# AlexanderVeselov/RayTracing

Measured on AMD Instinct MI355X. Metric: Mrays/s (all bounces+shadow), higher is better.
Workload: dtype f32

## Files before the change

### raytracing_amd/csrc/frame_kernels.h

```cpp
#pragma once
#include "raygen_kernels.h"
#include "trace_kernels.h"
#include "shade_kernels.h"

#define RT_FRAME_COUNT_STRIDE 136u

struct FrameArgs
{
    ShadeArgs shade;
    float4* o4[2]; float4* d4[2]; float4* thr[2];
    float4* hits;
    float4* sh_o4; float4* sh_d4; uint32_t* sh_aux;
    float4* radiance;
    uint2* spill;
    uint32_t* slow_list;
    uint32_t* wave_counts;
    rt_camera cam;
    float tan_half_fov;
    uint32_t max_bounces, drop_last, tune, tail_q, chunks_per_wave;
};

#ifndef RT_FRAME_WAVES
#define RT_FRAME_WAVES 5
#endif
// ... 51 lines not shown
        if (lane == 0) row[bounce] = n;
        if (lane == 0) row[130] = 0;
        w4_trace_body<false, 12, false, true, true>(sc, fa.o4[cur], fa.d4[cur], (const uint32_t*)nullptr, n, (uint32_t*)nullptr, fa.hits, log, fa.spill,
            fa.tune, my_slow, row + 130, row + 128, (unsigned long long*)nullptr, 0u, 0u, fa.tail_q, 1u, stack, w, G, first, S);
        {
            __threadfence_block();
            const uint32_t n_slow = row[130];
            for (uint32_t k = lane; k < n_slow; k += 64u)
            {
                const uint32_t i = my_slow[k];
                float4 hit;
                (void)v1_trace_ray<false>(sc, fa.o4[cur][i], fa.d4[cur][i], spill_push, spill_pop, hit);
                fa.hits[i] = hit;
            }
            if (lane == 0 && n_slow != 0u) row[129] += n_slow;
            __threadfence_block();
        }
        const unsigned long long t1 = wall_clock64();
        t_closest += t1 - t0;
        ShadeArgs a = fa.shade;
        a.in_o4 = fa.o4[cur]; a.in_d4 = fa.d4[cur]; a.in_thr = fa.thr[cur]; a.hits = fa.hits;
        a.bounce = bounce;
        a.emit_outgoing = (fa.drop_last && bounce >= fa.max_bounces) ? 0u : 1u;
        a.final_bounce = bounce >= fa.max_bounces ? 1u : 0u;
        a.count_in_ray = 1u;
        uint32_t n_next = 0, n_shadow = 0;
        for (uint32_t base = 0; base < n; base += 64u)
        {
            const uint32_t p = base + lane;
            bool want_shadow = false, want_next = false, no_block = false;
            uint32_t next_flag = 0, sh_entry = 0;
            float4 sh_o = make_float4(0, 0, 0, 0), sh_d = sh_o, nx_o = sh_o, nx_d = sh_o, nx_t = sh_o;
            if (p < n)
                shade_entry<FURNACE, BLUE, false, false>(sc, tile, a, index_of(p), want_shadow, want_next, no_block, next_flag, sh_o, sh_d, nx_o, nx_d, nx_t, sh_entry);
            const unsigned long long ms = __ballot(want_shadow), mn = __ballot(want_next);
            const unsigned long long lt = (1ull << lane) - 1ull;
            if (want_shadow)
            {
                const uint32_t i = index_of(n_shadow + (uint32_t)__popcll(ms & lt));
                fa.sh_o4[i] = sh_o; fa.sh_d4[i] = sh_d; fa.sh_aux[i] = sh_entry;
            }
            if (want_next)
            {
                const uint32_t i = index_of(n_next + (uint32_t)__popcll(mn & lt));
                fa.o4[cur ^ 1u][i] = nx_o; fa.d4[cur ^ 1u][i] = nx_d; fa.thr[cur ^ 1u][i] = nx_t;
            }
            n_shadow += (uint32_t)__popcll(ms);
            n_next += (uint32_t)__popcll(mn);
        }
        __threadfence_block();
        const unsigned long long t2 = wall_clock64();
        t_shade += t2 - t1;
        if (lane == 0) row[64u + bounce] = n_shadow;
        if (n_shadow != 0u)
        {
            if (lane == 0) row[130] = 0;
            w4_trace_body<true, 12, false, true, true>(sc, fa.sh_o4, fa.sh_d4, fa.sh_aux, n_shadow, (uint32_t*)nullptr, (float4*)nullptr, log, fa.spill,
                fa.tune, my_slow, row + 130, row + 128, (unsigned long long*)nullptr, 0u, 0u, fa.tail_q, 1u, stack, w, G, first, S);
            __threadfence_block();
            const uint32_t n_slow = row[130];
            for (uint32_t k = lane; k < n_slow; k += 64u)
            {
                const uint32_t i = my_slow[k];
                const float4 rd = fa.sh_d4[i];
                float4 hit;
                if (v1_trace_ray<true>(sc, fa.sh_o4[i], rd, spill_push, spill_pop, hit)) log_retract(log, fa.sh_aux[i], __float_as_uint(rd.w));
            }
            if (lane == 0 && n_slow != 0u) row[129] += n_slow;
            __threadfence_block();
        }
        t_shadow += wall_clock64() - t2;
        cur ^= 1u;
        n = n_next;
        if (n == 0u) break;
    }
    if (lane == 0)
    {
        row[131] = (uint32_t)t_closest; row[132] = (uint32_t)t_shade; row[133] = (uint32_t)t_shadow; row[134] = (uint32_t)(wall_clock64() - t_begin);
    }
    for (uint32_t p = lane; p < n_pixels; p += 64u)
    {
        const uint32_t id = index_of(p);
        const uint32_t c = log.cnt[id];
        if (c == 0u) continue;
        float4 r = fa.radiance[id];
        for (uint32_t k = 0; k < c; ++k)
        {
            const rt_rgb v = *reinterpret_cast<const rt_rgb*>(log.rlog + 3 * ((size_t)k * log.stride + id));
            r.x += v.x; r.y += v.y; r.z += v.z;
        }
        log.cnt[id] = 0;
        fa.radiance[id] = r;
    }
}

__global__ __launch_bounds__(256) void k_frame_sum(const uint32_t* __restrict__ wave_counts, uint32_t n_waves, uint32_t bounces, DCounters* __restrict__ counters)
{
    __shared__ uint32_t part[256];
    const uint32_t col = blockIdx.x;
    uint32_t s = 0;
    for (uint32_t wv = threadIdx.x; wv < n_waves; wv += 256u) s += wave_counts[(size_t)wv * RT_FRAME_COUNT_STRIDE + col];
    part[threadIdx.x] = s;
    __syncthreads();
    for (uint32_t step = 128u; step != 0u; step >>= 1)
    {
        if (threadIdx.x < step) part[threadIdx.x] += part[threadIdx.x + step];
        __syncthreads();
    }
    if (threadIdx.x == 0)
    {
        if (col < 64u) { if (col <= bounces) counters->queue[col] = part[0]; }
        else if (col < 128u) { if (col - 64u <= bounces) counters->shadow[col - 64u] = part[0]; }
        else if (col == 128u) counters->stack_spills += part[0];
        else counters->slow_rays += part[0];
    }
}
```

### raytracing_amd/csrc/kernels_common.h

```cpp
#pragma once
#include "device_math.h"
#include "rt_types.h"

#define RT_LEAF_BIT 0x80000000u
#define RT_EMPTY_REF 0xFFFFFFFFu
#define RT_TRACE_STACK_LDS 24
#define RT_TRACE_STACK_MAX 64

struct rt_rgb { float x, y, z; };
RT_DEV void log_store(float* __restrict__ rlog, size_t index, float x, float y, float z)
{
    rt_rgb v = {x, y, z};
    *reinterpret_cast<rt_rgb*>(rlog + 3 * index) = v;
}

typedef float rt_v4f __attribute__((ext_vector_type(4)));
RT_DEV float4 q_load(const float4* p) { const rt_v4f t = __builtin_nontemporal_load((const rt_v4f*)p); return make_float4(t.x, t.y, t.z, t.w); }
RT_DEV void q_store(float4* p, const float4& v) { const rt_v4f t = {v.x, v.y, v.z, v.w}; __builtin_nontemporal_store(t, (rt_v4f*)p); }

struct DLog
{
    float* rlog;
    uint32_t* cnt;
    uint32_t* ovf_slot;
    uint32_t stride;
    uint32_t inline_entries;
    uint32_t ovf_blocks;
};
RT_DEV size_t log_index(const DLog& L, uint32_t k, uint32_t id, uint32_t slot)
{
    if (k < L.inline_entries) return (size_t)k * L.stride + id;
    if (slot >= L.ovf_blocks) return ~(size_t)0;
    return (size_t)L.inline_entries * L.stride + (size_t)(k - L.inline_entries) * L.ovf_blocks + slot;
}
RT_DEV void log_put(const DLog& L, uint32_t k, uint32_t id, uint32_t slot, float x, float y, float z)
{
    const size_t i = log_index(L, k, id, slot);
    if (i != ~(size_t)0) log_store(L.rlog, i, x, y, z);
}

struct DScene
{
    const float4* nodes;
    const float4* tris_rt;
    const float4* tris_sh;
    const rt_packed_material* materials;
    const rt_texture* textures;
    const uint32_t* texture_data;
    const float4* lights;
    const float4* env;
    const float* gamma_lut;
    int env_w, env_h;
    uint32_t light_count;
    uint32_t root_ref;
    uint32_t entry_ref;
    const float4* wnodes;
    uint32_t w_entry_ref;
    const float4* wnodes_sh;
    uint32_t w_sh_entry_ref;
    float root_min[3];
    float root_max[3];
    const uint16_t* mat_tex16;
    const uint32_t* emissive;
    uint32_t emissive_count;
    uint32_t emissive_nee;
};

struct DTile
{
    uint32_t width, height;
// ... 39 lines not shown
```

### raytracing_amd/csrc/rt_hip.hip

```cpp
#include <hip/hip_runtime.h>
#include <stdio.h>
#include <stdlib.h>
#include <string.h>
#include <math.h>
#include <cmath>
#include <algorithm>
#include <string>
#include <vector>
#include <map>
#include <thread>
#include <atomic>
#include <array>
#include "rt_hip.h"
#include "kernels.h"
#include "own_bvh.h"
#include "treelet_order.h"
#include "tree_select.h"
#include "tree_rotate.h"
#include <chrono>
#include "wide_bvh.h"
#include "device_fold.h"
#include "refit.h"
#include "filters_host.h"
using namespace rtw;
// ... 1101 lines not shown
    HIPCHK(f->ctx, hipStreamWaitEvent(f->p->stream, f->p->ev_shadow[q], 0));
    f->p->shadow_in_flight[q] = false;
    return RT_OK;
}

bool side_on(const rt_frame* f) { return f->overlap_shadow != 0 && !(f->denoiser || f->aov != 0); }

int ensure_slots(rt_frame* f, uint32_t want)
{
    uint32_t cap = slot_cap(f);
    if (want > cap) want = cap;
    if (want <= f->slots && 2u * (f->max_bounces + 1u) <= f->log_entries && f->chunk_pixels == chunk_for(f, f->slots) &&
        (f->log_ovf_blocks != 0u) == log_is_compact(f, f->slots))
        return RT_OK;
    if (flush_log(f) != RT_OK || join_pipes(f) != RT_OK) return RT_ERROR;
    HIPCHK(f->ctx, hipStreamSynchronize(f->ctx->stream));
    uint32_t keep = f->slots < cap ? f->slots : cap;
    uint32_t n = want > keep ? want : keep;
    while (alloc_path_buffers(f, n) != RT_OK)
    {
        if (n == 1) return RT_ERROR;
        n = n > 2u * keep && keep > 0 ? n / 2u : (n > keep ? keep : n / 2u);
        if (n == 0) n = 1;
        f->slots_limit = n;
    }
    return RT_OK;
}

DLog dlog(const rt_frame* f)
{
    DLog L;
    L.rlog = f->p->rlog; L.cnt = f->p->cnt; L.ovf_slot = f->log_ovf_blocks ? f->p->ovf_slot : nullptr;
    L.stride = f->log_stride; L.inline_entries = f->log_inline; L.ovf_blocks = f->log_ovf_blocks;
    return L;
}

int ensure_whole_tile(rt_frame* f)
{
    if (f->chunk_pixels >= (f->n_local ? f->n_local : 1u)) return RT_OK;
    if (f->p->cur_slots != 0) return fail(f->ctx, "rt_generate_rays: the previous sample was not advanced (rt_advance_sample)");
    if (flush_log(f) != RT_OK || join_pipes(f) != RT_OK) return RT_ERROR;
    HIPCHK(f->ctx, hipStreamSynchronize(f->ctx->stream));
    return alloc_path_buffers(f, 1);
}

int flush_log(rt_frame* f, bool keep_open)
{
    rt_ctx* ctx = f->ctx;
    if (f->p->cur_slots == 0 || f->n_local == 0 || f->p->chunk_count == 0) { f->p->cur_slots = 0; return RT_OK; }
    if (f->p->shadow_pending)
        return fail(ctx, "radiance requested between rt_shade and rt_intersect_shadow (direct samples still tentative)");
    if (wait_shadow(f, 0) != RT_OK || wait_shadow(f, 1) != RT_OK) return RT_ERROR;
    uint32_t blocks = (f->p->chunk_count + 255u) / 256u;
    hipLaunchKernelGGL(k_flush, dim3(blocks), dim3(256), 0, f->p->stream, f->radiance + f->p->chunk_base, dlog(f),
        f->p->chunk_count, f->p->cur_slots, f->chunk_pixels, keep_open && f->log_ovf_blocks != 0u ? 1u : 0u, 0u);
    if (hipGetLastError() != hipSuccess) return fail(ctx, "k_flush launch failed");
    f->p->cur_slots = 0;
    return RT_OK;
}

}

static int sync_frame_streams(rt_frame* f)
{
    rt_ctx* ctx = f->ctx;
    for (PathPipe& q : f->ps)
    {
        if (q.stream && q.stream != ctx->stream) HIPCHK(ctx, hipStreamSynchronize(q.stream));
        if (q.side) HIPCHK(ctx, hipStreamSynchronize(q.side));
    }
    if (f->present_stream) HIPCHK(ctx, hipStreamSynchronize(f->present_stream));
    f->present_pending = false;
    return RT_OK;
}

extern "C" { static int deferred_materialize(rt_frame* f); }

namespace
{
int flush_log_keep(rt_frame* f)
{
    uint32_t keep = f->p->cur_slots;
    int rc = flush_log(f, true);
    f->p->cur_slots = keep;
    return rc;
}

template <class F>
// ... 1551 lines not shown
    rt_ctx* ctx = f->ctx;
    (void)hipSetDevice(ctx->device);
    if (bounce > RT_MAX_BOUNCES_LIMIT + 1) return fail(ctx, "rt_frame_debug_read_queue: bounce out of range");
    if (f->stage_chunks > 1) return fail(ctx, "rt_frame_debug_read_queue: the sample in flight is spread over several pipes (set RT_OPT_STAGE_PIPES to 1 for the debug readers)");
    if (f->deferred.active && deferred_materialize(f) != RT_OK) return RT_ERROR;
    if (f->p->side) HIPCHK(ctx, hipStreamSynchronize(f->p->side));
    DCounters h;
    HIPCHK(ctx, hipMemcpyAsync(&h, f->p->counters, sizeof(h), hipMemcpyDeviceToHost, ctx->stream));
    HIPCHK(ctx, hipStreamSynchronize(ctx->stream));
    uint32_t n = which == 0 ? h.queue[bounce] : h.shadow[bounce];
    if (n > f->log_stride) return fail(ctx, "rt_frame_debug_read_queue: corrupt counter");
    *count = n;
    if (n == 0) return RT_OK;
    if (!rays && !pixel_indices && !payload) return RT_OK;
    if (n > capacity) return fail(ctx, "rt_frame_debug_read_queue: the queue holds more entries than the caller's arrays");
    const float4* so = which == 0 ? f->p->o4[bounce & 1u] : f->p->sh_o4[bounce & 1u];
    const float4* sdir = which == 0 ? f->p->d4[bounce & 1u] : f->p->sh_d4[bounce & 1u];
    std::vector<float4> o(n), d(n), p(n);
    HIPCHK(ctx, hipMemcpy(o.data(), so, (size_t)n * 16, hipMemcpyDeviceToHost));
    HIPCHK(ctx, hipMemcpy(d.data(), sdir, (size_t)n * 16, hipMemcpyDeviceToHost));
    if (which == 0) HIPCHK(ctx, hipMemcpy(p.data(), f->p->thr[bounce & 1u], (size_t)n * 16, hipMemcpyDeviceToHost));
    for (uint32_t i = 0; i < n; ++i)
    {
        uint32_t pl;
        memcpy(&pl, &d[i].w, 4);
        uint32_t id = pl;
        uint32_t local_pix = f->p->chunk_base + id % (f->chunk_pixels ? f->chunk_pixels : 1);
        if (which == 1)
        {
            uint32_t entry = 0;
            HIPCHK(ctx, hipMemcpy(&entry, f->p->sh_aux[bounce & 1u] + i, 4, hipMemcpyDeviceToHost));
            p[i] = make_float4(0.0f, 0.0f, 0.0f, 0.0f);
            uint32_t oblk = 0;
            if (entry >= f->log_inline) HIPCHK(ctx, hipMemcpy(&oblk, f->p->ovf_slot + id, 4, hipMemcpyDeviceToHost));
            const size_t at = entry < f->log_inline ? (size_t)entry * f->log_stride + id
                                                    : (size_t)f->log_inline * f->log_stride + (size_t)(entry - f->log_inline) * f->log_ovf_blocks + oblk;
            HIPCHK(ctx, hipMemcpy(&p[i], f->p->rlog + 3u * at, 12, hipMemcpyDeviceToHost));
        }
        if (rays)
        {
            rays[i].origin.x = o[i].x; rays[i].origin.y = o[i].y; rays[i].origin.z = o[i].z; rays[i].origin.w = 0.0f;
            rays[i].direction.x = d[i].x; rays[i].direction.y = d[i].y; rays[i].direction.z = d[i].z;
            rays[i].direction.w = o[i].w;
        }
        if (pixel_indices)
        {
            uint32_t ly = local_pix / f->tile.width, px = local_pix - ly * f->tile.width;
            pixel_indices[i] = rt_frame_global_row(f, ly) * f->tile.width + px;
        }
        if (payload) { payload[i].x = p[i].x; payload[i].y = p[i].y; payload[i].z = p[i].z; payload[i].w = 0.0f; }
    }
    return RT_OK;
}

int rt_frame_debug_read_hits(rt_frame* f, rt_hit* hits, uint32_t count)
{
    if (!f || !hits) return fail(nullptr, "rt_frame_debug_read_hits: NULL argument");
    rt_ctx* ctx = f->ctx;
    (void)hipSetDevice(ctx->device);
    if (count > f->log_stride) return fail(ctx, "rt_frame_debug_read_hits: count too large");
    if (f->stage_chunks > 1) return fail(ctx, "rt_frame_debug_read_hits: the sample in flight is spread over several pipes (set RT_OPT_STAGE_PIPES to 1 for the debug readers)");
    if (f->deferred.active && deferred_materialize(f) != RT_OK) return RT_ERROR;
    std::vector<float4> h(count ? count : 1);
    HIPCHK(ctx, hipStreamSynchronize(ctx->stream));
    HIPCHK(ctx, hipMemcpy(h.data(), f->p->hits, (size_t)count * 16, hipMemcpyDeviceToHost));
    for (uint32_t i = 0; i < count; ++i)
    {
        hits[i].bc.x = h[i].x; hits[i].bc.y = h[i].y;
// ... 80 lines not shown
```

### raytracing_amd/csrc/samples_ahead_impl.h

```cpp
#pragma once

#define RT_AHEAD_QUIET 3u

static bool ahead_bank_idle(const AheadBank& b) { return b.next >= b.n; }

static int ahead_holds(const rt_frame* f, uint32_t s)
{
    if (!f->ahead || !f->ahead_opt) return -1;
    const Ahead& A = *f->ahead;
    if (A.scene != f->ctx->scene_uploads || memcmp(&A.camera, &f->camera, sizeof(rt_camera)) != 0) return -1;
    for (int i = 0; i < 2; ++i)
        if (A.bank[i].h && !ahead_bank_idle(A.bank[i]) && A.bank[i].base + A.bank[i].next == s) return i;
    return -1;
}

static uint32_t ahead_depth(const rt_frame* f)
{
    const uint64_t n = f->n_local ? f->n_local : 1u;
    uint64_t k = f->ahead_opt & 0xFFu;
    if (k == 0) return 0;
    if (k == 1 || k == 255) { k = (32000000ull + n - 1) / n; if (k > 64) k = 64; }
    const uint64_t budget = f->state_limit_mb ? ((uint64_t)f->state_limit_mb << 20) : (64ull << 30);
    const uint64_t per_sample = 2ull * n * (11u * 16u + 5u * 4u + 12u * 2u * (f->max_bounces + 1u));
    if (k * per_sample > budget) k = budget / per_sample;
// ... 78 lines not shown
    for (uint32_t bounce = 0; bounce <= h->max_bounces && rc == RT_OK; ++bounce)
    {
        if (rt_shade(h, bounce) != RT_OK) rc = RT_ERROR;
        else if (h->side_active && bounce < h->max_bounces && rt_intersect(h, bounce + 1u) != RT_OK) rc = RT_ERROR;
        else if (rt_intersect_shadow(h, bounce) != RT_OK) rc = RT_ERROR;
        else if (!h->side_active && bounce < h->max_bounces && rt_intersect(h, bounce + 1u) != RT_OK) rc = RT_ERROR;
    }
    if (rc == RT_OK && (wait_shadow(h, 0) != RT_OK || wait_shadow(h, 1) != RT_OK)) rc = RT_ERROR;
    h->fused = false;
    if (rc == RT_OK && hipEventRecord(b.done, st) != hipSuccess) rc = fail(ctx, "RT_OPT_SAMPLES_AHEAD: recording a batch's end failed");
    if (rc != RT_OK)
    {
        (void)hipGetLastError();
        (void)sync_frame_streams(h);
        (void)hipMemsetAsync(h->ps[0].cnt, 0, (size_t)h->log_stride * sizeof(uint32_t), st);
        h->ps[0].cur_slots = 0; h->ps[0].shadow_pending = false; h->ps[0].shadow_in_flight[0] = h->ps[0].shadow_in_flight[1] = false;
        b.n = b.next = 0;
        return RT_ERROR;
    }
    b.base = base; b.n = n; b.next = 0;
    A.camera = f->camera;
    A.scene = ctx->scene_uploads;
    A.last_n = n;
    A.launched += n;
    return RT_OK;
}

static int ahead_consume(rt_frame* f, int i)
{
    rt_ctx* ctx = f->ctx;
    AheadBank& b = f->ahead->bank[i];
    rt_frame* h = b.h;
    HIPCHK(ctx, hipStreamWaitEvent(ctx->stream, b.done, 0));
    const uint32_t blocks = (f->n_local + 255u) / 256u;
    hipLaunchKernelGGL(k_flush, dim3(blocks), dim3(256), 0, ctx->stream, f->radiance, dlog(h), f->n_local, 1u, h->chunk_pixels, 0u, b.next);
    HIPCHK(ctx, hipGetLastError());
    ++b.next;
    ++f->sample_count;
    ++f->ahead->consumed;
    if (ahead_bank_idle(b)) h->ps[0].cur_slots = 0;
    return RT_OK;
}

static void ahead_schedule(rt_frame* f, bool starting)
{
    if (!ahead_wanted(f)) return;
    if (ahead_configure(f) != RT_OK) { (void)hipGetLastError(); f->ahead_opt = 0; return; }
    Ahead& A = *f->ahead;
    if (A.depth < 2u) return;
    const uint32_t s = f->sample_count;
    if (!starting && ahead_holds(f, s) < 0 && !(ahead_bank_idle(A.bank[0]) && ahead_bank_idle(A.bank[1]))) return;
    for (int i = 0; i < 2; ++i)
    {
        if (!ahead_bank_idle(A.bank[i])) continue;
        uint32_t end = s;
        for (const AheadBank& o : A.bank) if (!ahead_bank_idle(o)) end = std::max(end, o.base + o.n);
        const uint32_t n = ahead_bank_idle(A.bank[i ^ 1]) ? 2u : std::min(A.depth, 2u * std::max(1u, A.last_n));
        if (end > 0xFFFFFFFFu - n) return;
        if (ahead_launch(f, i, end, n) != RT_OK) { (void)hipGetLastError(); return; }
        if (starting) return;
    }
}

static void ahead_discard(rt_frame* f)
{
    if (!f || !f->ahead) return;
    Ahead& A = *f->ahead;
    A.quiet = 0;
// ... 44 lines not shown
```

### raytracing_amd/csrc/shade_kernels.h

```cpp
#pragma once
#include "kernels_common.h"

#include "material_kernels.h"

__global__ void k_fill_gamma_lut(float* __restrict__ lut)
{
    float v = (float)threadIdx.x / 255.0f;
    lut[threadIdx.x] = rt_powf(cl_min(cl_max(v, 0.0f), 1.0f), 2.2f);
}

RT_DEV float IorToF0(float ior_incident, float ior_transmitted)
{
    float result = (ior_transmitted - ior_incident) / (ior_transmitted + ior_incident);
    return result * result;
}

RT_DEV f3 FresnelSchlick(f3 f0, float h_dot_o)
{
    float p = rt_powf(1.0f - h_dot_o, 5.0f);
    return F3(f0.x + (1.0f - f0.x) * p, f0.y + (1.0f - f0.y) * p, f0.z + (1.0f - f0.z) * p);
}

RT_DEV float GGX_D(float alpha, float n_dot_h)
{
// ... 229 lines not shown
    }
    __syncthreads();
    idx_a = s_base[0] + s_cnt[0][key_a % KEYS][wave] + rank_a;
    idx_b = s_base[1] + s_cnt[1][key_b % KEYS][wave] + rank_b;
}

struct ShadeArgs
{
    const float4* in_o4; const float4* in_d4; const float4* in_thr; const float4* hits;
    float4* out_o4; float4* out_d4; float4* out_thr;
    float4* sh_o4; float4* sh_d4; uint32_t* sh_aux;
    DLog log;
    const uint8_t* bn_sobol; const uint8_t* bn_scramble; const uint8_t* bn_rank;
    DCounters* counters;
    uint32_t bounce, sample_base, emit_outgoing, n_local;
    uint32_t pix_base;
    uint32_t partition;
    uint32_t final_bounce;
    uint32_t count_in_ray;
};

RT_DEV float SampleBlueNoise(const ShadeArgs& a, uint32_t px, uint32_t py, uint32_t sample_index, uint32_t dim)
{
    int pixel_i = (int)px & 127, pixel_j = (int)py & 127;
    int sampleIndex = (int)sample_index & 255, sampleDimension = (int)dim & 255;
    int ridx = sampleDimension + (pixel_i + pixel_j * 128) * 8;
    int rank = ridx < 128 * 128 * 8 ? (int)a.bn_rank[ridx] : 0;
    int rankedSampleIndex = sampleIndex ^ rank;
    int value = (int)a.bn_sobol[sampleDimension + rankedSampleIndex * 256];
    value = value ^ (int)a.bn_scramble[(sampleDimension % 8) + (pixel_i + pixel_j * 128) * 8];
    return (0.5f + (float)value) / 256.0f;
}

template <bool FURNACE, bool BLUE, bool NEE, bool COMPACT>
RT_DEV void shade_entry(const DScene& sc, const DTile& tile, const ShadeArgs& a, const uint32_t i, bool& want_shadow, bool& want_next, bool& no_block,
    uint32_t& next_flag, float4& sh_o, float4& sh_d, float4& nx_o, float4& nx_d, float4& nx_t, uint32_t& sh_entry)
{
    float4 hit = a.hits[i];
    float4 rd = a.in_d4[i];
    uint32_t prim = __float_as_uint(hit.z);
    uint32_t id = __float_as_uint(rd.w);
    uint32_t slot = id / a.n_local;
    uint32_t pix = id - slot * a.n_local;
    uint32_t sample_idx = a.sample_base + slot;
    float4 thr4 = a.in_thr[i];
    uint32_t nlog = a.count_in_ray ? (__float_as_uint(thr4.w) & 0x7FFFFFFFu) : a.log.cnt[id];
    uint32_t oblk = RT_EMPTY_REF;
    if (COMPACT && nlog + 1u >= a.log.inline_entries) oblk = a.log.ovf_slot[id];
    no_block = oblk == RT_EMPTY_REF;
    auto put = [&](float x, float y, float z)
    {
        if (COMPACT) log_put(a.log, nlog, id, oblk, x, y, z);
        else log_store(a.log.rlog, (size_t)nlog * a.log.stride + id, x, y, z);
    };
    const bool prev_delta = NEE && (__float_as_uint(thr4.w) >> 31) != 0u;
    f3 hit_throughput = F3(thr4.x, thr4.y, thr4.z);

    if (prim == RT_INVALID_ID)
    {
        f3 sky = FURNACE ? F3s(0.5f) : SampleSky(sc, F3(rd.x, rd.y, rd.z));
        f3 add = sky * hit_throughput;
        put(add.x, add.y, add.z);
        ++nlog;
    }
    else
    {
        f3 incoming = F3(-rd.x, -rd.y, -rd.z);
        uint32_t lp = a.pix_base + pix;
        uint32_t ly = lp / tile.width;
        uint32_t px = lp - ly * tile.width;
        uint32_t py = tile_global_row(tile, ly);

        const float4* tp = sc.tris_sh + (size_t)prim * 8;
        float4 q0 = tp[0], q1 = tp[1], q2 = tp[2], q3 = tp[3], q4 = tp[4], q5 = tp[5], q6 = tp[6];
        f3 p1 = xyz(q0), p2 = xyz(q1), p3 = xyz(q2);
        f3 n1 = xyz(q3), n2 = xyz(q4), n3 = xyz(q5);
        float bu = hit.x, bv = hit.y;
        float w0 = 1.0f - bu - bv;
        f3 position = p1 * w0 + p2 * bu + p3 * bv;
        f3 geometry_normal = normalize3(cross3(p2 - p1, p3 - p1));
        f2 texcoord;
        texcoord.x = q0.w * w0 + q2.w * bu + q4.w * bv;
        texcoord.y = q1.w * w0 + q3.w * bu + q5.w * bv;
        f3 normal = normalize3(n1 * w0 + n2 * bu + n3 * bv);

        Material material;
// ... 79 lines not shown
            sh_o = make_float4(so.x, so.y, so.z, distance_to_light);
            sh_d = make_float4(outgoing.x, outgoing.y, outgoing.z, __uint_as_float(id));
            sh_entry = nlog;
            if (want_shadow)
            {
                put(lsamp.x, lsamp.y, lsamp.z);
                ++nlog;
            }
        }

        if (a.emit_outgoing != 0)
        {
            f2 s;
            s.x = draw(2);
            s.y = draw(3);
            float s1 = draw(1);
            float pdf = 0.0f;
            f3 outgoing;
            float offset;
            bool delta;
            f3 bxdf = SampleBxdf<FURNACE>(s1, s, material, normal, incoming, outgoing, pdf, offset, delta);
            if (NEE && delta) next_flag = 0x80000000u;
            f3 throughput = F3s(0.0f);
            if ((double)pdf > 0.0) throughput = bxdf / pdf;
            f3 new_thr = hit_throughput * throughput;
            want_next = (double)pdf > 0.0;
            f3 oo = position + geometry_normal * RT_EPS * offset;
            nx_o = make_float4(oo.x, oo.y, oo.z, RT_MAX_RENDER_DIST);
            nx_d = make_float4(outgoing.x, outgoing.y, outgoing.z, rd.w);
            nx_t = make_float4(new_thr.x, new_thr.y, new_thr.z, 0.0f);
        }
    }
    nx_t.w = __uint_as_float(nlog | next_flag);
    if (!a.count_in_ray || ((!want_next || a.final_bounce) && nlog != 0u)) a.log.cnt[id] = nlog;
}

template <bool FURNACE, bool BLUE, bool NEE = false, bool COMPACT = false>
__global__ __launch_bounds__(RT_SHADE_BLOCK) __attribute__((amdgpu_waves_per_eu(NEE ? 5 : RT_SHADE_WAVES))) void k_shade(DScene sc, DTile tile, ShadeArgs a)
{
    const uint32_t count = a.counters->queue[a.bounce];
    {
        const uint32_t g = blockIdx.x * RT_SHADE_BLOCK + threadIdx.x;
        if (g < 16)
        {
            const uint32_t fl = g < 8 ? 0u : 1u + (a.bounce & 1u);
            a.counters->head[fl][g & 7] = 0; a.counters->slow_head[fl][g & 7] = 0;
            if ((g & 7) == 0) a.counters->slow_count[fl] = 0;
        }
    }
    if (blockIdx.x * RT_SHADE_BLOCK >= count) return;
    uint32_t i = blockIdx.x * RT_SHADE_BLOCK + threadIdx.x;
    if (a.partition)
    {
        __shared__ uint16_t s_perm[RT_SHADE_BLOCK];
        __shared__ uint32_t s_hit[RT_SHADE_BLOCK / 64], s_miss[RT_SHADE_BLOCK / 64];
        const uint32_t lane = threadIdx.x & 63u, wave = threadIdx.x >> 6;
        const bool valid = i < count;
        const bool is_miss = valid && __float_as_uint(a.hits[valid ? i : 0u].z) == RT_INVALID_ID;
        const unsigned long long mh = __ballot(valid && !is_miss), mm = __ballot(is_miss);
        if (lane == 0) { s_hit[wave] = (uint32_t)__popcll(mh); s_miss[wave] = (uint32_t)__popcll(mm); }
        __syncthreads();
        uint32_t hits_before = 0, miss_before = 0, hits_total = 0;
        for (uint32_t w = 0; w < RT_SHADE_BLOCK / 64; ++w)
        {
            hits_total += s_hit[w];
            if (w < wave) { hits_before += s_hit[w]; miss_before += s_miss[w]; }
        }
// ... 12 lines not shown
    float4 sh_o = make_float4(0, 0, 0, 0), sh_d = sh_o, nx_o = sh_o, nx_d = sh_o, nx_t = sh_o;
    uint32_t sh_entry = 0;

    if (active) shade_entry<FURNACE, BLUE, NEE, COMPACT>(sc, tile, a, i, want_shadow, want_next, no_block, next_flag, sh_o, sh_d, nx_o, nx_d, nx_t, sh_entry);
    if (COMPACT && 2u * (a.bounce + 1u) + 1u >= a.log.inline_entries && !a.final_bounce)
    {
        const bool want_block = want_next && no_block && (__float_as_uint(nx_t.w) & 0x7FFFFFFFu) + 1u >= a.log.inline_entries;
        unsigned long long wm = __ballot(want_block);
        if (wm != 0ull)
        {
            const uint32_t lane = threadIdx.x & 63u;
            const uint32_t home = blockIdx.x * (RT_SHADE_BLOCK / 64u) + (threadIdx.x >> 6);
            uint32_t n_pools = RT_LOG_SUBPOOLS;
            while (n_pools > 1u && a.log.ovf_blocks / n_pools < 32u) n_pools >>= 1;
            const uint32_t share = a.log.ovf_blocks / n_pools, last_share = a.log.ovf_blocks - share * (n_pools - 1u);
            uint32_t got = RT_EMPTY_REF;
            for (uint32_t attempt = 0; attempt < (n_pools < 8u ? n_pools : 8u) && wm != 0ull; ++attempt)
            {
                const uint32_t pool = (home + attempt * (n_pools > 8u ? 9u : 1u)) & (n_pools - 1u);
                uint32_t base = 0;
                const int first = __builtin_ctzll(wm);
                if ((int)lane == first) base = atomicAdd(&a.counters->log_ovf_next[pool], (uint32_t)__popcll(wm));
                base = (uint32_t)__shfl((int)base, first, 64);
                if (want_block && got == RT_EMPTY_REF)
                {
                    const uint32_t k = base + (uint32_t)__popcll(wm & ((1ull << lane) - 1ull));
                    if (k < (pool == n_pools - 1u ? last_share : share)) got = pool * share + k;
                }
                wm = __ballot(want_block && got == RT_EMPTY_REF);
            }
            if (want_block)
            {
                if (got == RT_EMPTY_REF) a.counters->log_ovf_flag = 1u;
                a.log.ovf_slot[__float_as_uint(nx_d.w)] = got;
            }
        }
    }

    uint32_t sidx, nidx;
    if (a.partition & 2u)
    {
        const uint32_t key_s = (sh_d.x < 0.0f ? 1u : 0u) | (sh_d.y < 0.0f ? 2u : 0u) | (sh_d.z < 0.0f ? 4u : 0u);
        const uint32_t key_n = (nx_d.x < 0.0f ? 1u : 0u) | (nx_d.y < 0.0f ? 2u : 0u) | (nx_d.z < 0.0f ? 4u : 0u);
        block_append2_keyed<8>(want_shadow, key_s, want_next, key_n, &a.counters->shadow[a.bounce], &a.counters->queue[a.bounce + 1], sidx, nidx);
    }
    else
        block_append2(want_shadow, want_next, &a.counters->shadow[a.bounce], &a.counters->queue[a.bounce + 1], sidx, nidx);
    if (want_shadow)
    {
        a.sh_o4[sidx] = sh_o;
        a.sh_d4[sidx] = sh_d;
        a.sh_aux[sidx] = sh_entry;
    }
    if (want_next)
    {
        a.out_o4[nidx] = nx_o;
        a.out_d4[nidx] = nx_d;
        a.out_thr[nidx] = nx_t;
    }
}

__global__ __launch_bounds__(256) void k_flush(float4* __restrict__ radiance, DLog log, uint32_t n_pixels, uint32_t n_slots, uint32_t id_stride,
    uint32_t keep_open, uint32_t first_slot)
{
    uint32_t p = blockIdx.x * 256u + threadIdx.x;
    if (p >= n_pixels) return;
    float4 r = radiance[p];
    for (uint32_t slot = first_slot; slot < first_slot + n_slots; ++slot)
    {
        uint32_t id = slot * id_stride + p;
        uint32_t c = log.cnt[id];
        const uint32_t oblk = c > log.inline_entries ? log.ovf_slot[id] : 0u;
        for (uint32_t k = 0; k < c; ++k)
        {
            const size_t at = log_index(log, k, id, oblk);
            if (at == ~(size_t)0) continue;
            const rt_rgb v = *reinterpret_cast<const rt_rgb*>(log.rlog + 3 * at);
            r.x += v.x; r.y += v.y; r.z += v.z;
            if (keep_open) log_store(log.rlog, at, 0.0f, 0.0f, 0.0f);
        }
        if (c && !keep_open) log.cnt[id] = 0;
    }
    radiance[p] = r;
}
```

### raytracing_amd/csrc/trace_kernels.h

```cpp
#pragma once
#include "kernels_common.h"


RT_DEV bool box_test(float bminx, float bminy, float bminz, float bmaxx, float bmaxy, float bmaxz, f3 org, f3 inv,
    float t_min, float t_max, float& entry)
{
    float t0x = (bminx - org.x) * inv.x, t0y = (bminy - org.y) * inv.y, t0z = (bminz - org.z) * inv.z;
    float t1x = (bmaxx - org.x) * inv.x, t1y = (bmaxy - org.y) * inv.y, t1z = (bmaxz - org.z) * inv.z;
    float lox = cl_min(t0x, t1x), loy = cl_min(t0y, t1y), loz = cl_min(t0z, t1z);
    float hix = cl_max(t0x, t1x), hiy = cl_max(t0y, t1y), hiz = cl_max(t0z, t1z);
    float tmin = cl_max(cl_max(cl_max(lox, loy), loz), t_min);
    float tmax = cl_min(cl_min(cl_min(hix, hiy), hiz), t_max);
    entry = tmin;
    return tmax >= tmin;
}

RT_DEV float hw_min(float a, float b) { float r; asm("v_min_f32 %0, %1, %2" : "=v"(r) : "v"(a), "v"(b)); return r; }
RT_DEV float hw_max(float a, float b) { float r; asm("v_max_f32 %0, %1, %2" : "=v"(r) : "v"(a), "v"(b)); return r; }
RT_DEV float hw_min3(float a, float b, float c) { float r; asm("v_min3_f32 %0, %1, %2, %3" : "=v"(r) : "v"(a), "v"(b), "v"(c)); return r; }
RT_DEV float hw_max3(float a, float b, float c) { float r; asm("v_max3_f32 %0, %1, %2, %3" : "=v"(r) : "v"(a), "v"(b), "v"(c)); return r; }

#define RT_NODE_C0(q0, q1, q2) (q0).x, (q0).y, (q2).x, (q0).z, (q0).w, (q2).y
#define RT_NODE_C1(q0, q1, q2) (q1).x, (q1).y, (q2).z, (q1).z, (q1).w, (q2).w

RT_DEV bool box_test_fast(float bminx, float bminy, float bminz, float bmaxx, float bmaxy, float bmaxz, f3 org, f3 inv,
    float t_min, float t_max, float& entry)
{
    float t0x = (bminx - org.x) * inv.x, t0y = (bminy - org.y) * inv.y, t0z = (bminz - org.z) * inv.z;
    float t1x = (bmaxx - org.x) * inv.x, t1y = (bmaxy - org.y) * inv.y, t1z = (bmaxz - org.z) * inv.z;
    float lox = hw_min(t0x, t1x), loy = hw_min(t0y, t1y), loz = hw_min(t0z, t1z);
    float hix = hw_max(t0x, t1x), hiy = hw_max(t0y, t1y), hiz = hw_max(t0z, t1z);
    float tmin = hw_max(hw_max3(lox, loy, loz), t_min);
    float tmax = hw_min(hw_min3(hix, hiy, hiz), t_max);
    entry = tmin;
    return tmax >= tmin;
}

RT_DEV void log_retract(const DLog& L, uint32_t entry, uint32_t id)
{
    const uint32_t slot = entry < L.inline_entries ? 0u : L.ovf_slot[id];
    log_put(L, entry, id, slot, 0.0f, 0.0f, 0.0f);
}

template <bool SHADOW, class Push, class Pop>
RT_DEV bool v1_trace_ray(const DScene& sc, const float4 ro, const float4 rd, Push&& push, Pop&& pop, float4& hit_out)
{
    f3 org = F3(ro.x, ro.y, ro.z), dir = F3(rd.x, rd.y, rd.z);
    const float t_min = 0.0f;
    float t_max = ro.w;
    f3 inv = F3(1.0f / dir.x, 1.0f / dir.y, 1.0f / dir.z);
    uint32_t sign_bits = (inv.x < 0.0f ? 1u : 0u) | (inv.y < 0.0f ? 2u : 0u) | (inv.z < 0.0f ? 4u : 0u);

    uint32_t hit_prim = RT_INVALID_ID;
    float hit_u = 0.0f, hit_v = 0.0f, hit_t = 0.0f;
    bool occluded = false;

    int sp = 0;
    uint32_t ref = sc.root_ref;
    float entry;
    bool alive = box_test(sc.root_min[0], sc.root_min[1], sc.root_min[2], sc.root_max[0], sc.root_max[1],
        sc.root_max[2], org, inv, t_min, t_max, entry);

    while (alive)
    {
        bool need_pop;
        if (ref & RT_LEAF_BIT)
        {
            uint32_t prim = ref & ~RT_LEAF_BIT;
            bool last;
            do
            {
                const float4* tp = sc.tris_rt + (size_t)prim * 4;
                float4 a = tp[0], b = tp[1], cc = tp[2];
                last = a.w != 0.0f;
// ... 584 lines not shown
            }
            if (SHADOW && accepted) ref = RT_IDLE_REF;
            else if (last) pop();
            else ref = (RT_LEAF_BIT | RT_LEAF_CONT_BIT) | (prim + 1u);
        }
    };
    auto node_step = [&](const float4 q0, const float4 q1, const float4 q2, const float4 q3)
    {
        if (TIMELINE) ++tl_steps;
        uint32_t r[4];
        float e[4];
        w4_test_slots<SHADOW>(q0, q1, q2, q3, org, inv, sign_bits, octant4, t_min, t_max, r, e);
        const bool v0 = e[0] < INF, v1 = e[1] < INF, v2 = e[2] < INF, v3 = e[3] < INF;
        if (v3 && (v0 || v1 || v2)) push(r[3], e[3]);
        if (v2 && (v0 || v1)) push(r[2], e[2]);
        if (v1 && v0) push(r[1], e[1]);
        if (v0) ref = r[0];
        else if (v1) ref = r[1];
        else if (v2) ref = r[2];
        else if (v3) ref = r[3];
        else pop();
    };

    for (;;)
    {
        const unsigned long long idle_m = __ballot(ref == RT_IDLE_REF);
        if ((chunk_mode && !(TAIL && chunk_refill)) ? idle_m == ~0ull : idle_m != 0ull)
        {
            if (ref == RT_IDLE_REF && ray_i != RT_INVALID_ID)
            {
                if (SHADOW)
                {
                    if (hit_prim != RT_INVALID_ID)
                        log_retract(log, log_entry, payload);
                }
                else
                    q_store(hits + ray_i, make_float4(hit_u, hit_v, __uint_as_float(hit_prim), t_max));
                if (TIMELINE)
                {
                    const unsigned long long dt = wall_clock64() - tl_t0;
                    if (dt > tl_max_ticks) { tl_max_ticks = dt; tl_steps_of_slowest = tl_steps; }
                    tl_max_steps = tl_steps > tl_max_steps ? tl_steps : tl_max_steps;
                }
                ray_i = RT_INVALID_ID;
            }
            if (!pool.exhausted)
            {
                if (PRIVATE)
                {
                    const unsigned long long need = __ballot(ref == RT_IDLE_REF && ray_i == RT_INVALID_ID);
                    const uint32_t avail = count - chunk_next;
                    const uint32_t rank = __builtin_amdgcn_mbcnt_hi((uint32_t)(need >> 32), __builtin_amdgcn_mbcnt_lo((uint32_t)need, 0u));
                    const uint32_t n = (uint32_t)__popcll(need);
                    if (ref == RT_IDLE_REF && ray_i == RT_INVALID_ID && rank < avail)
                    {
                        const uint32_t p = chunk_next + rank;
                        ray_i = (priv_first + (p >> 6) * priv_stride) * 64u + (p & 63u);
                    }
                    chunk_next += n < avail ? n : avail;
                    if (chunk_next >= count) pool.exhausted = true;
                }
                else if (TAIL && chunk_mode && chunk_refill)
                {
                    const uint32_t rb = xcd * per < count ? xcd * per : count;
                    const uint32_t re = (xcd + 1u) * per < count ? (xcd + 1u) * per : count;
                    unsigned long long need = __ballot(ref == RT_IDLE_REF && ray_i == RT_INVALID_ID);
                    while (need != 0ull)
// ... 159 lines not shown
```

Measured before the change: 6839.

## Use pixel-major radiance log layout and add transposed LDS-staged flush kernel

Reorders the per-sample radiance log so that columns are pixel-major (id*slots+slot) when not in ahead mode, replacing the integer division for slot with a precomputed magic multiply. A new flush kernel assigns 16 threads per pixel across a slot window, stages log entries into LDS via a block prefix sum, and then reduces them per pixel. The aim is to make flush reads of a pixel's samples contiguous and to cut division cost. In exchange, writes during shading become strided across slots, and the new flush path adds extra synchronisation.

```diff
diff --git a/raytracing_amd/csrc/frame_kernels.h b/raytracing_amd/csrc/frame_kernels.h
--- a/raytracing_amd/csrc/frame_kernels.h
+++ b/raytracing_amd/csrc/frame_kernels.h
@@ -107,7 +107,7 @@
             uint32_t next_flag = 0, sh_entry = 0;
             float4 sh_o = make_float4(0, 0, 0, 0), sh_d = sh_o, nx_o = sh_o, nx_d = sh_o, nx_t = sh_o;
             if (p < n)
-                shade_entry<FURNACE, BLUE, false, false>(sc, tile, a, index_of(p), want_shadow, want_next, no_block, next_flag, sh_o, sh_d, nx_o, nx_d, nx_t, sh_entry);
+                shade_entry<FURNACE, BLUE, false, false, true>(sc, tile, a, index_of(p), want_shadow, want_next, no_block, next_flag, sh_o, sh_d, nx_o, nx_d, nx_t, sh_entry);
             const unsigned long long ms = __ballot(want_shadow), mn = __ballot(want_next);
             const unsigned long long lt = (1ull << lane) - 1ull;
             if (want_shadow)
@@ -139,7 +139,7 @@
                 const uint32_t i = my_slow[k];
                 const float4 rd = fa.sh_d4[i];
                 float4 hit;
-                if (v1_trace_ray<true>(sc, fa.sh_o4[i], rd, spill_push, spill_pop, hit)) log_retract(log, fa.sh_aux[i], __float_as_uint(rd.w));
+                if (v1_trace_ray<true>(sc, fa.sh_o4[i], rd, spill_push, spill_pop, hit)) log_retract<true>(log, fa.sh_aux[i], __float_as_uint(rd.w));
             }
             if (lane == 0 && n_slow != 0u) row[129] += n_slow;
             __threadfence_block();
@@ -156,15 +156,16 @@
     for (uint32_t p = lane; p < n_pixels; p += 64u)
     {
         const uint32_t id = index_of(p);
-        const uint32_t c = log.cnt[id];
+        const uint32_t col = log_column(log, id, 0u);
+        const uint32_t c = log.cnt[col];
         if (c == 0u) continue;
         float4 r = fa.radiance[id];
         for (uint32_t k = 0; k < c; ++k)
         {
-            const rt_rgb v = *reinterpret_cast<const rt_rgb*>(log.rlog + 3 * ((size_t)k * log.stride + id));
+            const rt_rgb v = *reinterpret_cast<const rt_rgb*>(log.rlog + 3 * ((size_t)k * log.stride + col));
             r.x += v.x; r.y += v.y; r.z += v.z;
         }
-        log.cnt[id] = 0;
+        log.cnt[col] = 0;
         fa.radiance[id] = r;
     }
 }
diff --git a/raytracing_amd/csrc/kernels_common.h b/raytracing_amd/csrc/kernels_common.h
--- a/raytracing_amd/csrc/kernels_common.h
+++ b/raytracing_amd/csrc/kernels_common.h
@@ -26,16 +26,38 @@
     uint32_t stride;
     uint32_t inline_entries;
     uint32_t ovf_blocks;
+    uint32_t chunk_pixels;
+    uint32_t div_mul, div_sh;
+    uint32_t col_id, col_slot;
 };
-RT_DEV size_t log_index(const DLog& L, uint32_t k, uint32_t id, uint32_t slot)
+#define RT_HD __host__ __device__ __forceinline__
+RT_HD uint32_t log_slot(const DLog& L, uint32_t id)
 {
-    if (k < L.inline_entries) return (size_t)k * L.stride + id;
+    const uint32_t t = (uint32_t)(((unsigned long long)id * L.div_mul) >> 32);
+    return (t + ((id - t) >> (L.div_sh & 0xFFu))) >> (L.div_sh >> 8);
+}
+RT_HD uint32_t log_column(const DLog& L, uint32_t id, uint32_t slot) { return id * L.col_id + slot * L.col_slot; }
+RT_HD uint32_t log_column(const DLog& L, uint32_t id) { return log_column(L, id, log_slot(L, id)); }
+inline void log_set_layout(DLog& L, uint32_t chunk_pixels, uint32_t slots, bool pixel_major)
+{
+    const uint32_t d = chunk_pixels ? chunk_pixels : 1u;
+    uint32_t l = 0;
+    while (l < 32u && (1ull << l) < d) ++l;
+    L.chunk_pixels = d;
+    L.div_mul = (uint32_t)((((1ull << l) - d) << 32) / d + 1ull);
+    L.div_sh = (l < 1u ? l : 1u) | ((l > 1u ? l - 1u : 0u) << 8);
+    L.col_id = pixel_major ? (slots ? slots : 1u) : 1u;
+    L.col_slot = pixel_major ? 1u - d * L.col_id : 0u;
+}
+RT_DEV size_t log_index(const DLog& L, uint32_t k, uint32_t col, uint32_t slot)
+{
+    if (k < L.inline_entries) return (size_t)k * L.stride + col;
     if (slot >= L.ovf_blocks) return ~(size_t)0;
     return (size_t)L.inline_entries * L.stride + (size_t)(k - L.inline_entries) * L.ovf_blocks + slot;
 }
-RT_DEV void log_put(const DLog& L, uint32_t k, uint32_t id, uint32_t slot, float x, float y, float z)
+RT_DEV void log_put(const DLog& L, uint32_t k, uint32_t col, uint32_t slot, float x, float y, float z)
 {
-    const size_t i = log_index(L, k, id, slot);
+    const size_t i = log_index(L, k, col, slot);
     if (i != ~(size_t)0) log_store(L.rlog, i, x, y, z);
 }
 
diff --git a/raytracing_amd/csrc/rt_hip.hip b/raytracing_amd/csrc/rt_hip.hip
--- a/raytracing_amd/csrc/rt_hip.hip
+++ b/raytracing_amd/csrc/rt_hip.hip
@@ -1157,6 +1157,7 @@
     DLog L;
     L.rlog = f->p->rlog; L.cnt = f->p->cnt; L.ovf_slot = f->log_ovf_blocks ? f->p->ovf_slot : nullptr;
     L.stride = f->log_stride; L.inline_entries = f->log_inline; L.ovf_blocks = f->log_ovf_blocks;
+    log_set_layout(L, f->chunk_pixels, f->slots, f->ahead_owner == nullptr);
     return L;
 }
 
@@ -1176,9 +1177,7 @@
     if (f->p->shadow_pending)
         return fail(ctx, "radiance requested between rt_shade and rt_intersect_shadow (direct samples still tentative)");
     if (wait_shadow(f, 0) != RT_OK || wait_shadow(f, 1) != RT_OK) return RT_ERROR;
-    uint32_t blocks = (f->p->chunk_count + 255u) / 256u;
-    hipLaunchKernelGGL(k_flush, dim3(blocks), dim3(256), 0, f->p->stream, f->radiance + f->p->chunk_base, dlog(f),
-        f->p->chunk_count, f->p->cur_slots, f->chunk_pixels, keep_open && f->log_ovf_blocks != 0u ? 1u : 0u, 0u);
+    launch_flush(f->p->stream, f->radiance + f->p->chunk_base, dlog(f), f->p->chunk_count, f->p->cur_slots, keep_open && f->log_ovf_blocks != 0u ? 1u : 0u, 0u);
     if (hipGetLastError() != hipSuccess) return fail(ctx, "k_flush launch failed");
     f->p->cur_slots = 0;
     return RT_OK;
@@ -2796,8 +2795,9 @@
             HIPCHK(ctx, hipMemcpy(&entry, f->p->sh_aux[bounce & 1u] + i, 4, hipMemcpyDeviceToHost));
             p[i] = make_float4(0.0f, 0.0f, 0.0f, 0.0f);
             uint32_t oblk = 0;
-            if (entry >= f->log_inline) HIPCHK(ctx, hipMemcpy(&oblk, f->p->ovf_slot + id, 4, hipMemcpyDeviceToHost));
-            const size_t at = entry < f->log_inline ? (size_t)entry * f->log_stride + id
+            const uint32_t col = log_column(dlog(f), id);
+            if (entry >= f->log_inline) HIPCHK(ctx, hipMemcpy(&oblk, f->p->ovf_slot + col, 4, hipMemcpyDeviceToHost));
+            const size_t at = entry < f->log_inline ? (size_t)entry * f->log_stride + col
                                                     : (size_t)f->log_inline * f->log_stride + (size_t)(entry - f->log_inline) * f->log_ovf_blocks + oblk;
             HIPCHK(ctx, hipMemcpy(&p[i], f->p->rlog + 3u * at, 12, hipMemcpyDeviceToHost));
         }
diff --git a/raytracing_amd/csrc/samples_ahead_impl.h b/raytracing_amd/csrc/samples_ahead_impl.h
--- a/raytracing_amd/csrc/samples_ahead_impl.h
+++ b/raytracing_amd/csrc/samples_ahead_impl.h
@@ -134,8 +134,7 @@
     AheadBank& b = f->ahead->bank[i];
     rt_frame* h = b.h;
     HIPCHK(ctx, hipStreamWaitEvent(ctx->stream, b.done, 0));
-    const uint32_t blocks = (f->n_local + 255u) / 256u;
-    hipLaunchKernelGGL(k_flush, dim3(blocks), dim3(256), 0, ctx->stream, f->radiance, dlog(h), f->n_local, 1u, h->chunk_pixels, 0u, b.next);
+    launch_flush(ctx->stream, f->radiance, dlog(h), f->n_local, 1u, 0u, b.next);
     HIPCHK(ctx, hipGetLastError());
     ++b.next;
     ++f->sample_count;
diff --git a/raytracing_amd/csrc/shade_kernels.h b/raytracing_amd/csrc/shade_kernels.h
--- a/raytracing_amd/csrc/shade_kernels.h
+++ b/raytracing_amd/csrc/shade_kernels.h
@@ -285,7 +285,7 @@
     return (0.5f + (float)value) / 256.0f;
 }
 
-template <bool FURNACE, bool BLUE, bool NEE, bool COMPACT>
+template <bool FURNACE, bool BLUE, bool NEE, bool COMPACT, bool ONE_SLOT = false>
 RT_DEV void shade_entry(const DScene& sc, const DTile& tile, const ShadeArgs& a, const uint32_t i, bool& want_shadow, bool& want_next, bool& no_block,
     uint32_t& next_flag, float4& sh_o, float4& sh_d, float4& nx_o, float4& nx_d, float4& nx_t, uint32_t& sh_entry)
 {
@@ -293,18 +293,19 @@
     float4 rd = a.in_d4[i];
     uint32_t prim = __float_as_uint(hit.z);
     uint32_t id = __float_as_uint(rd.w);
-    uint32_t slot = id / a.n_local;
+    uint32_t slot = ONE_SLOT ? 0u : log_slot(a.log, id);
     uint32_t pix = id - slot * a.n_local;
+    const uint32_t col = log_column(a.log, id, slot);
     uint32_t sample_idx = a.sample_base + slot;
     float4 thr4 = a.in_thr[i];
-    uint32_t nlog = a.count_in_ray ? (__float_as_uint(thr4.w) & 0x7FFFFFFFu) : a.log.cnt[id];
+    uint32_t nlog = a.count_in_ray ? (__float_as_uint(thr4.w) & 0x7FFFFFFFu) : a.log.cnt[col];
     uint32_t oblk = RT_EMPTY_REF;
-    if (COMPACT && nlog + 1u >= a.log.inline_entries) oblk = a.log.ovf_slot[id];
+    if (COMPACT && nlog + 1u >= a.log.inline_entries) oblk = a.log.ovf_slot[col];
     no_block = oblk == RT_EMPTY_REF;
     auto put = [&](float x, float y, float z)
     {
-        if (COMPACT) log_put(a.log, nlog, id, oblk, x, y, z);
-        else log_store(a.log.rlog, (size_t)nlog * a.log.stride + id, x, y, z);
+        if (COMPACT) log_put(a.log, nlog, col, oblk, x, y, z);
+        else log_store(a.log.rlog, (size_t)nlog * a.log.stride + col, x, y, z);
     };
     const bool prev_delta = NEE && (__float_as_uint(thr4.w) >> 31) != 0u;
     f3 hit_throughput = F3(thr4.x, thr4.y, thr4.z);
@@ -450,7 +451,7 @@
         }
     }
     nx_t.w = __uint_as_float(nlog | next_flag);
-    if (!a.count_in_ray || ((!want_next || a.final_bounce) && nlog != 0u)) a.log.cnt[id] = nlog;
+    if (!a.count_in_ray || ((!want_next || a.final_bounce) && nlog != 0u)) a.log.cnt[col] = nlog;
 }
 
 template <bool FURNACE, bool BLUE, bool NEE = false, bool COMPACT = false>
@@ -529,7 +530,7 @@
             if (want_block)
             {
                 if (got == RT_EMPTY_REF) a.counters->log_ovf_flag = 1u;
-                a.log.ovf_slot[__float_as_uint(nx_d.w)] = got;
+                a.log.ovf_slot[log_column(a.log, __float_as_uint(nx_d.w))] = got;
             }
         }
     }
@@ -557,26 +558,106 @@
     }
 }
 
-__global__ __launch_bounds__(256) void k_flush(float4* __restrict__ radiance, DLog log, uint32_t n_pixels, uint32_t n_slots, uint32_t id_stride,
-    uint32_t keep_open, uint32_t first_slot)
+__global__ __launch_bounds__(256) void k_flush(float4* __restrict__ radiance, DLog log, uint32_t n_pixels, uint32_t n_slots, uint32_t keep_open, uint32_t first_slot)
 {
     uint32_t p = blockIdx.x * 256u + threadIdx.x;
     if (p >= n_pixels) return;
     float4 r = radiance[p];
     for (uint32_t slot = first_slot; slot < first_slot + n_slots; ++slot)
     {
-        uint32_t id = slot * id_stride + p;
-        uint32_t c = log.cnt[id];
-        const uint32_t oblk = c > log.inline_entries ? log.ovf_slot[id] : 0u;
+        const uint32_t col = log_column(log, slot * log.chunk_pixels + p, slot);
+        uint32_t c = log.cnt[col];
+        const uint32_t oblk = c > log.inline_entries ? log.ovf_slot[col] : 0u;
         for (uint32_t k = 0; k < c; ++k)
         {
-            const size_t at = log_index(log, k, id, oblk);
+            const size_t at = log_index(log, k, col, oblk);
             if (at == ~(size_t)0) continue;
             const rt_rgb v = *reinterpret_cast<const rt_rgb*>(log.rlog + 3 * at);
             r.x += v.x; r.y += v.y; r.z += v.z;
             if (keep_open) log_store(log.rlog, at, 0.0f, 0.0f, 0.0f);
         }
-        if (c && !keep_open) log.cnt[id] = 0;
+        if (c && !keep_open) log.cnt[col] = 0;
     }
     radiance[p] = r;
 }
+
+#define RT_FLUSH_PIXELS 16u
+#define RT_FLUSH_WINDOW 16u
+#define RT_FLUSH_LDS 1024u
+__global__ __launch_bounds__(256) void k_flush_t(float4* __restrict__ radiance, DLog log, uint32_t n_pixels, uint32_t n_slots, uint32_t keep_open, uint32_t first_slot)
+{
+    static_assert(RT_FLUSH_PIXELS * RT_FLUSH_WINDOW == 256u, "one column per thread");
+    __shared__ float s_v[RT_FLUSH_LDS * 3u];
+    __shared__ uint32_t s_off[257], s_cnt[256], s_blk[256], s_wave[4];
+    const uint32_t t = threadIdx.x, lane = t & 63u, wave = t >> 6;
+    const uint32_t p = blockIdx.x * RT_FLUSH_PIXELS + t / RT_FLUSH_WINDOW, w = t % RT_FLUSH_WINDOW;
+    const uint32_t my_p = blockIdx.x * RT_FLUSH_PIXELS + t;
+    const bool adder = t < RT_FLUSH_PIXELS && my_p < n_pixels;
+    const uint32_t end_slot = first_slot + n_slots;
+    float4 r = make_float4(0, 0, 0, 0);
+    if (adder) r = radiance[my_p];
+    uint32_t c_next = (p < n_pixels && first_slot + w < end_slot) ? log.cnt[p * log.col_id + first_slot + w] : 0u;
+    for (uint32_t s0 = first_slot; s0 < end_slot; s0 += RT_FLUSH_WINDOW)
+    {
+        const uint32_t col = p * log.col_id + s0 + w;
+        const uint32_t c_raw = c_next;
+        c_next = (p < n_pixels && s0 + RT_FLUSH_WINDOW + w < end_slot) ? log.cnt[col + RT_FLUSH_WINDOW] : 0u;
+        const uint32_t oblk = c_raw > log.inline_entries ? log.ovf_slot[col] : 0u;
+        const uint32_t c = (c_raw > log.inline_entries && oblk >= log.ovf_blocks) ? log.inline_entries : c_raw;
+        uint32_t incl = c;
+        for (uint32_t d = 1; d < 64u; d <<= 1)
+        {
+            const uint32_t up = (uint32_t)__shfl_up((int)incl, d, 64);
+            if (lane >= d) incl += up;
+        }
+        if (lane == 63u) s_wave[wave] = incl;
+        __syncthreads();
+        uint32_t base = 0, total = 0;
+        for (uint32_t i = 0; i < 4u; ++i) { const uint32_t n = s_wave[i]; total += n; if (i < wave) base += n; }
+        const uint32_t off = base + incl - c;
+        s_off[t] = off; s_cnt[t] = c; s_blk[t] = oblk;
+        if (t == 255u) s_off[256] = total;
+        const bool in_lds = total <= RT_FLUSH_LDS;
+        if (in_lds)
+            for (uint32_t k = 0; k < c; ++k)
+            {
+                const size_t at = log_index(log, k, col, oblk);
+                const rt_rgb v = *reinterpret_cast<const rt_rgb*>(log.rlog + 3 * at);
+                float* const d = s_v + 3u * (off + k);
+                d[0] = v.x; d[1] = v.y; d[2] = v.z;
+                if (keep_open) log_store(log.rlog, at, 0.0f, 0.0f, 0.0f);
+            }
+        if (c_raw && !keep_open) log.cnt[col] = 0;
+        __syncthreads();
+        if (adder)
+        {
+            if (in_lds)
+            {
+                const uint32_t j1 = s_off[(t + 1u) * RT_FLUSH_WINDOW];
+                for (uint32_t j = s_off[t * RT_FLUSH_WINDOW]; j < j1; ++j) { r.x += s_v[3u * j]; r.y += s_v[3u * j + 1u]; r.z += s_v[3u * j + 2u]; }
+            }
+            else
+                for (uint32_t i = 0; i < RT_FLUSH_WINDOW; ++i)
+                {
+                    const uint32_t mc = my_p * log.col_id + s0 + i, n = s_cnt[t * RT_FLUSH_WINDOW + i], blk = s_blk[t * RT_FLUSH_WINDOW + i];
+                    for (uint32_t k = 0; k < n; ++k)
+                    {
+                        const size_t at = log_index(log, k, mc, blk);
+                        const rt_rgb v = *reinterpret_cast<const rt_rgb*>(log.rlog + 3 * at);
+                        r.x += v.x; r.y += v.y; r.z += v.z;
+                        if (keep_open) log_store(log.rlog, at, 0.0f, 0.0f, 0.0f);
+                    }
+                }
+        }
+        __syncthreads();
+    }
+    if (adder) radiance[my_p] = r;
+}
+
+inline void launch_flush(hipStream_t stream, float4* radiance, const DLog& log, uint32_t n_pixels, uint32_t n_slots, uint32_t keep_open, uint32_t first_slot)
+{
+    if (log.col_id > 1u && n_slots >= RT_FLUSH_WINDOW / 2u)
+        hipLaunchKernelGGL(k_flush_t, dim3((n_pixels + RT_FLUSH_PIXELS - 1u) / RT_FLUSH_PIXELS), dim3(256), 0, stream, radiance, log, n_pixels, n_slots, keep_open, first_slot);
+    else
+        hipLaunchKernelGGL(k_flush, dim3((n_pixels + 255u) / 256u), dim3(256), 0, stream, radiance, log, n_pixels, n_slots, keep_open, first_slot);
+}
diff --git a/raytracing_amd/csrc/trace_kernels.h b/raytracing_amd/csrc/trace_kernels.h
--- a/raytracing_amd/csrc/trace_kernels.h
+++ b/raytracing_amd/csrc/trace_kernels.h
@@ -36,10 +36,12 @@
     return tmax >= tmin;
 }
 
+template <bool ONE_SLOT = false>
 RT_DEV void log_retract(const DLog& L, uint32_t entry, uint32_t id)
 {
-    const uint32_t slot = entry < L.inline_entries ? 0u : L.ovf_slot[id];
-    log_put(L, entry, id, slot, 0.0f, 0.0f, 0.0f);
+    const uint32_t col = ONE_SLOT ? log_column(L, id, 0u) : log_column(L, id);
+    const uint32_t slot = entry < L.inline_entries ? 0u : L.ovf_slot[col];
+    log_put(L, entry, col, slot, 0.0f, 0.0f, 0.0f);
 }
 
 template <bool SHADOW, class Push, class Pop>
@@ -690,7 +692,7 @@
                 if (SHADOW)
                 {
                     if (hit_prim != RT_INVALID_ID)
-                        log_retract(log, log_entry, payload);
+                        log_retract<PRIVATE>(log, log_entry, payload);
                 }
                 else
                     q_store(hits + ray_i, make_float4(hit_u, hit_v, __uint_as_float(hit_prim), t_max));
```

Result: no change. 6818 (-0.3%).
